# Jakoebly/marl-sc

Measured on AMD Instinct MI355X. Metric: env-steps/sec (agents×envs×steps) at 1/2/4/8 MI355X; CPU ref same host, higher is better.
Workload: dtype int32 state, u64 PCG64, f64 rewards, f32 obs; 1 GPU; InventoryEnvironment.step x 32768 envs/GPU, 8 agents x 64 regions x 5 SKUs (BASELINE configs[2]; configs[3] when N>1); n_envs_per_gpu=32768, agents=8, regions=64, skus=5, episode_length=100, obs_dim_local=34, obs_normalization=meanstd_custom, parallelism=env-shard x1

## Files before the change

### marl-sc_amd/csrc/alloc_kernels.hip

```cpp
#include <hip/hip_runtime.h>
#include <math.h>

#include "env.hpp"
#include "kcommon.hpp"

namespace msc {

#ifndef MSC_AL_CH
#define MSC_AL_CH 8
#endif
constexpr int AL_CH = MSC_AL_CH;
template <int K>
hipError_t launch_alloc_lane_k(const EnvConst& c, const DevEnv* d, const StepIO& io, hipStream_t st);
#ifndef MSC_AL_PRIO
#define MSC_AL_PRIO 3
#endif
#ifndef MSC_AL_PRIO2
#define MSC_AL_PRIO2 1
#endif
#ifndef MSC_AL_PRIO_TAIL
#define MSC_AL_PRIO_TAIL 0
#endif
#ifndef MSC_AL_TAIL_WIN
#define MSC_AL_TAIL_WIN 0
#endif

struct AlLds {
  int rec, inv, shh, qs, out, pen, tab, hm, cl, total;
  __host__ __device__ static AlLds make(int MWL, int MW, int K, int R, bool tab, bool SH) {
    AlLds L{};
    int o = 0;
    L.rec = o; o += AL_CH * ((1 + K + 7) / 8) * 64 * 4;
    L.inv = o; o += MWL * K * 64;
    L.shh = o; o += SH ? MWL * K * 64 : 0;
    L.qs = o;  o += MWL * 64;
    o = (o + 3) & ~3;
    L.out = o; o += MWL * 64 * 2;
    L.pen = o; o += MWL * 64 * 2;
    L.tab = o; o += tab ? (R | 1) * MW * 4 : 0;
    L.hm = o;  o += R;
    L.cl = o;  o += R;
    L.total = o;
    return L;
  }
};
constexpr size_t AL_TAB_MAX = 32 * 1024;

template <int K, int MW, bool DBG, bool TAB, bool SH, bool EXACT, int LPE>
__global__ __launch_bounds__(64) void alloc_lane_kernel(const DevEnv* __restrict__ dp, StepIO io) {
  static_assert(LPE == 1 || LPE == 2 || LPE == 4, "lanes per env");
  static_assert(MW % LPE == 0, "warehouses per lane");
  constexpr int MWL = MW / LPE, EPB = 64 / LPE, LSH = LPE == 1 ? 0 : LPE == 2 ? 1 : 2;
  constexpr int SENT = 0x7fff;
  const EnvConst& c = dp->c;
  const EnvState& s = dp->s;
  const int W = EXACT ? MW : c.W, R = c.R, WK = W * K;
  const int64_t E = c.E;
  const int lane = threadIdx.x, jl = lane & (LPE - 1);
  const int64_t e = (int64_t)blockIdx.x * EPB + (lane >> LSH);
  const bool ev = e < E;
  const msc_step_info info = io.info;
  constexpr bool dbg = DBG;
  constexpr int NVR = Rec<K>::NV;
  if (MSC_AL_PRIO > 0) __builtin_amdgcn_s_setprio(MSC_AL_PRIO);
  auto gw = [&](int i) { return i * LPE + jl; };

  extern __shared__ __attribute__((aligned(16))) int32_t al_lds[];
  const AlLds L = AlLds::make(MWL, MW, K, R, TAB, SH);
  int32_t* Linv = al_lds + L.inv + lane;
  int32_t* Lshh = al_lds + L.shh + lane;
  uint4* Lrec = reinterpret_cast<uint4*>(al_lds + L.rec) + lane;
  double* Lout = reinterpret_cast<double*>(al_lds + L.out) + lane;
  double* Lpen = reinterpret_cast<double*>(al_lds + L.pen) + lane;
  int32_t* Lqs = al_lds + L.qs + lane;
  MSC_GLOBAL int32_t* const incp = gp(s.inc);
  const double2* Ltab = TAB ? reinterpret_cast<const double2*>(al_lds + L.tab) : nullptr;
  const int RS = R | 1;
  const uint32_t* Lhm = reinterpret_cast<const uint32_t*>(al_lds + L.hm);
  const int32_t* Lcl = al_lds + L.cl;
  {
    double2* tw_ = reinterpret_cast<double2*>(al_lds + L.tab);
    if constexpr (TAB) {
      for (int i = lane; i < R * MW; i += 64) {
        const int w = i / R, r = i % R;
        tw_[w * RS + r] = w < W ? make_double2(c.ofT[r * W + w], c.ovT[r * W + w]) : make_double2(0.0, 0.0);
      }
    }
    uint32_t* hm_ = reinterpret_cast<uint32_t*>(al_lds + L.hm);
    int32_t* cl_ = al_lds + L.cl;
    for (int i = lane; i < R; i += 64) {
      hm_[i] = c.home_mask[i];
      cl_[i] = c.closest[i];
    }
  }
  auto tab_at = [&](int r, int w) -> double2 {
    if constexpr (TAB) return Ltab[w * RS + r];
    else return make_double2(gp(c.ofT)[r * W + w], gp(c.ovT)[r * W + w]);
  };

  uint32_t stock[K];
#pragma unroll
  for (int sk = 0; sk < K; sk++) stock[sk] = 0u;
  int invv[MWL][K];
  {
    const int64_t ec = ev ? e : 0;
#pragma unroll
    for (int i = 0; i < MWL; i++) {
      const int w = gw(i), wc = w < W ? w : W - 1;
#pragma unroll
      for (int sk = 0; sk < K; sk++) invv[i][sk] = gp(s.inv)[(int64_t)(wc * K + sk) * E + ec];
    }
  }
#pragma unroll
  for (int i = 0; i < MWL; i++) {
    const int w = gw(i);
#pragma unroll
    for (int sk = 0; sk < K; sk++) {
      const int v = (ev && w < W) ? invv[i][sk] : 0;
      Linv[(i * K + sk) * 64] = v;
      if (SH) Lshh[(i * K + sk) * 64] = 0;
      stock[sk] |= v > 0 ? (1u << i) : 0u;
    }
    Lout[i * 64] = 0.0;
    Lpen[i * 64] = 0.0;
    Lqs[i * 64] = 0;
  }
  __syncthreads();

  const OrderSrc osrc = order_src<NVR>(c, s, io, ev ? e : 0);
  const int n_orders = ev ? osrc.n : 0;
  const int64_t base = ev ? osrc.base : 0, nstep = osrc.nstep, vstep = osrc.vstep;
  const MSC_GLOBAL uint4* src = gp(osrc.src);
  if (dbg && ev && jl == 0 && info.n_orders) info.n_orders[e] = n_orders;
  int wmax = n_orders;
#pragma unroll
  for (int o = 32; o >= 1; o >>= 1) {
    const int v = __shfl_xor(wmax, o);
    wmax = v > wmax ? v : wmax;
  }
  wmax = __builtin_amdgcn_readfirstlane(wmax);

  const int maxwh = c.max_wh, lost_type = c.lost_type, pps = c.pen_per_sku;
  const double alpha = sgpr_d(c.alpha);
  double skw[K], penk[K];
#pragma unroll
  for (int sk = 0; sk < K; sk++) {
    skw[sk] = sgpr_d(c.skw[sk]);
    penk[sk] = sgpr_d(pps ? c.pen[sk] : c.pen_scalar);
  }

  const uint32_t ownw = LPE == 1 ? ~0u : (LPE == 2 ? 0x55555555u : 0x11111111u) << jl;
  int cur = -1, lost_cnt = 0;
  uint32_t hm = 0;
  int hw = -1;
  uint32_t smask = 0;
  int rtot = 0;
  int u[K], dsum[K], shc[K];
#pragma unroll
  for (int sk = 0; sk < K; sk++) u[sk] = dsum[sk] = shc[sk] = 0;
  MSC_GLOBAL int32_t* const shhp = gp(s.sc_shh);
  if (!SH && ev)
    for (int i = 0; i < MWL; i++) {
      const int w = gw(i);
      if (w < W)
        for (int sk = 0; sk < K; sk++) shhp[(int64_t)(w * K + sk) * E + e] = 0;
    }

  auto add_pen = [&](int i, double wt, double upen) {
    Lpen[i * 64] += wt * upen;
    if (dbg && info.lost_sales)
#pragma unroll
      for (int sk = 0; sk < K; sk++) info.lost_sales[e * WK + gw(i) * K + sk] += wt * (double)u[sk];
  };
  auto finalize = [&](int r) {
    if (lost_cnt > 0) {
      double upen = 0.0;
#pragma unroll
      for (int sk = 0; sk < K; sk++) upen += pps ? (double)u[sk] * penk[sk] : ((double)u[sk] * skw[sk]) * penk[sk];
      if (lost_type == MSC_LOST_COST) {
        if constexpr (LPE == 1) {
          double lw = 0.0;
#pragma unroll
          for (int sk = 0; sk < K; sk++) lw += (double)u[sk] * skw[sk];
          double lg[16], mx = -INFINITY;
#pragma unroll
          for (int w = 0; w < 16; w++) {
            lg[w] = -INFINITY;
            if (w < MW && w < W) {
              const double2 t = tab_at(r, w);
              lg[w] = -(t.x * (double)lost_cnt + t.y * lw) / alpha;
              mx = lg[w] > mx ? lg[w] : mx;
            }
          }
          double ex[16];
#pragma unroll
          for (int w = 0; w < 16; w++) ex[w] = (w < MW && w < W) ? exp(lg[w] - mx) : 0.0;
          const double sum = np_sum_f64_16(ex, W);
#pragma unroll
          for (int w = 0; w < MW; w++) {
            const double wt = w < W ? ex[w] / sum : 0.0;
            if (wt != 0.0) add_pen(w, wt, upen);
          }
        }
      } else if (lost_type == MSC_LOST_SHIPMENT && rtot > 0) {
        const double dt = (double)rtot;
        for (uint32_t m = smask; m != 0u; m &= m - 1u) {
          const int i = __builtin_ctz(m);
          add_pen(i, (double)Lqs[i * 64] / dt, upen);
        }
      } else {
        const int cw = Lcl[r];
        if ((cw & (LPE - 1)) == jl) add_pen(cw >> LSH, 1.0, upen);
      }
    }
    for (uint32_t m = smask; m != 0u; m &= m - 1u) Lqs[__builtin_ctz(m) * 64] = 0;
    if (!SH && hw >= 0 && (hw & (LPE - 1)) == jl)
#pragma unroll
      for (int sk = 0; sk < K; sk++) shhp[(int64_t)(hw * K + sk) * E + e] = shc[sk];
    for (uint32_t m = hm & ownw; m != 0u; m &= m - 1u) {
      const int w = __builtin_ctz(m);
#pragma unroll
      for (int sk = 0; sk < K; sk++) incp[(int64_t)(w * K + sk) * E + e] = dsum[sk];
    }
    if (dbg && jl == 0) {
#pragma unroll
      for (int sk = 0; sk < K; sk++) {
        if (info.demand_per_region) info.demand_per_region[(e * R + r) * K + sk] = dsum[sk];
        if (info.unfulfilled_demands) info.unfulfilled_demands[(e * R + r) * K + sk] = u[sk];
      }
      if (info.lost_order_counts) info.lost_order_counts[e * R + r] = lost_cnt;
    }
  };

  uint4 nxt[AL_CH][NVR];
  auto fetch = [&](int win) {
#pragma unroll
    for (int j = 0; j < AL_CH; j++) {
      const int oi = win * AL_CH + j;
#pragma unroll
      for (int v = 0; v < NVR; v++)
        nxt[j][v] = oi < n_orders ? gload4(src, base + oi * nstep + v * vstep) : make_uint4(0u, 0u, 0u, 0u);
    }
  };
  auto publish = [&]() {
#pragma unroll
    for (int j = 0; j < AL_CH; j++)
#pragma unroll
      for (int v = 0; v < NVR; v++) Lrec[(j * NVR + v) * 64] = nxt[j][v];
  };
  fetch(0);
  publish();
  fetch(1);

  const int aps = __builtin_amdgcn_readfirstlane(c.chain_prio ? 16 : c.al_psplit);
  const int psplit = MSC_AL_PRIO > 0 && aps < 16 ? (wmax * aps) >> 4 : -1;
  const bool tail_on = LPE == 1 && __builtin_amdgcn_readfirstlane(c.al_tail) != 0;
  int tail_at = -1;
  int oi = 0;
  for (; oi <= wmax; oi++) {
    if constexpr (LPE == 1) {
      if (tail_on && oi < wmax && (MSC_AL_TAIL_WIN == 0 || oi % AL_CH == 0)) {
        uint32_t any = 0u;
#pragma unroll
        for (int sk = 0; sk < K; sk++) any |= stock[sk];
        if (__builtin_amdgcn_ballot_w64(any != 0u && oi < n_orders) == 0ull) {
          tail_at = oi;
          break;
        }
      }
    }
    if (oi == psplit) __builtin_amdgcn_s_setprio(MSC_AL_PRIO2);
    const int jw = oi % AL_CH;
    if (jw == 0 && oi > 0) {
      publish();
      fetch(oi / AL_CH + 1);
    }
    union {
      uint4 v[NVR];
      uint16_t h[8 * NVR];
    } ur;
#pragma unroll
    for (int v = 0; v < NVR; v++) ur.v[v] = Lrec[(jw * NVR + v) * 64];
    const int r = oi < n_orders ? (int)ur.h[0] : -1;
    if (r != cur) {
#ifndef MSC_AL_ABL_NOFIN
      if (cur >= 0) finalize(cur);
#endif
      cur = r;
      lost_cnt = 0;
#pragma unroll
      for (int sk = 0; sk < K; sk++) u[sk] = dsum[sk] = 0;
      hm = r >= 0 ? Lhm[r] : 0u;
      hw = hm != 0u ? __builtin_ctz(hm) : -1;
      smask = 0u;
      rtot = 0;
#pragma unroll
      for (int sk = 0; sk < K; sk++) shc[sk] = 0;
    }
    if (oi < n_orders) {
    int d[K], rem[K];
    double tw = 0.0;
#pragma unroll
    for (int sk = 0; sk < K; sk++) {
      d[sk] = ur.h[1 + sk];
      rem[sk] = d[sk];
      dsum[sk] += d[sk];
      tw += (double)d[sk] * skw[sk];
    }
    double2 trow[MWL];
#pragma unroll
    for (int i = 0; i < MWL; i++) trow[i] = tab_at(r, TAB ? gw(i) : (gw(i) < W ? gw(i) : W - 1));
    double cost[MWL];
#pragma unroll
    for (int i = 0; i < MWL; i++) cost[i] = gw(i) < W ? trow[i].x + trow[i].y * tw : INFINITY;
    int used = 0;
    bool open = true;
    while (open) {
      uint32_t cand = 0u;
#pragma unroll
      for (int sk = 0; sk < K; sk++) cand |= rem[sk] > 0 ? stock[sk] : 0u;
      if (LPE == 1 && cand == 0u) {
        open = false;
      } else {
      double best = INFINITY;
      int b = LPE == 1 ? 0 : SENT;
#pragma unroll
      for (int i = 0; i < MWL; i++) {
        const bool take = ((cand >> i) & 1u) && cost[i] < best;
        best = take ? cost[i] : best;
        b = take ? gw(i) : b;
      }
      if constexpr (LPE > 1) {
        auto mn = [&](double ob, int o) {
          const bool t = ob < best || (ob == best && o < b);
          best = t ? ob : best;
          b = t ? o : b;
        };
        mn(dpp_x<0>(best), dpp_x<0>(b));
        if constexpr (LPE == 4) mn(dpp_x<1>(best), dpp_x<1>(b));
      }
      if (LPE > 1 && b == SENT) {
        open = false;
      } else {
      const bool own = (b & (LPE - 1)) == jl;
      const int ib = b >> LSH;
      int iv[K], sh[K];
#pragma unroll
      for (int sk = 0; sk < K; sk++) {
        iv[sk] = Linv[(ib * K + sk) * 64];
        sh[sk] = SH ? Lshh[(ib * K + sk) * 64] : 0;
      }
      const bool home_b = (hm >> b) & 1u;
      const double out_b = Lout[ib * 64];
      const int qs_b = Lqs[ib * 64];
      const double2 tb = tab_at(r, b);
      int f[K], fs = 0;
#pragma unroll
      for (int sk = 0; sk < K; sk++) f[sk] = own ? (rem[sk] < iv[sk] ? rem[sk] : iv[sk]) : 0;
      if constexpr (LPE > 1) {
        constexpr int NP = (K + 1) / 2;
        uint32_t pk[NP];
#pragma unroll
        for (int p = 0; p < NP; p++)
          pk[p] = (uint32_t)f[2 * p] | (2 * p + 1 < K ? (uint32_t)f[2 * p + 1] << 16 : 0u);
#pragma unroll
        for (int p = 0; p < NP; p++) {
          pk[p] |= (uint32_t)dpp_x<0>((int)pk[p]);
          if constexpr (LPE == 4) pk[p] |= (uint32_t)dpp_x<1>((int)pk[p]);
        }
#pragma unroll
        for (int sk = 0; sk < K; sk++) f[sk] = (int)((pk[sk / 2] >> (16 * (sk & 1))) & 0xffffu);
      }
      double fw = 0.0;
      bool done = true;
#pragma unroll
      for (int sk = 0; sk < K; sk++) {
        rem[sk] -= f[sk];
        done &= rem[sk] <= 0;
        fs += f[sk];
        fw += (double)f[sk] * skw[sk];
        if (!SH) shc[sk] += home_b ? f[sk] : 0;
      }
      const double oc = fw == tw ? best : tb.x + tb.y * fw;
      if (own) {
#pragma unroll
        for (int sk = 0; sk < K; sk++) {
          const int left = iv[sk] - f[sk];
          stock[sk] &= left > 0 ? ~0u : ~(1u << ib);
          Linv[(ib * K + sk) * 64] = left;
          if (SH) Lshh[(ib * K + sk) * 64] = sh[sk] + (home_b ? f[sk] : 0);
        }
        Lout[ib * 64] = out_b + oc;
        Lqs[ib * 64] = qs_b + fs;
        smask |= 1u << ib;
        if (dbg) {
#pragma unroll
          for (int sk = 0; sk < K; sk++) {
            if (info.shipment_quantities_by_sku) info.shipment_quantities_by_sku[((e * W + b) * R + r) * K + sk] += f[sk];
            if (info.fulfilled_per_warehouse) info.fulfilled_per_warehouse[e * WK + b * K + sk] += f[sk];
          }
          if (info.shipment_counts) info.shipment_counts[(e * W + b) * R + r] += 1;
          if (info.shipment_quantities) info.shipment_quantities[(e * W + b) * R + r] += fs;
        }
      }
      rtot += fs;
      used++;
      open = !(done || used >= maxwh);
#ifdef MSC_AL_ABL_ONEROUND
      open = false;
#endif
      }
      }
    }
    int remor = 0;
#pragma unroll
    for (int sk = 0; sk < K; sk++) {
      remor |= rem[sk];
      u[sk] += rem[sk];
    }
    lost_cnt += remor != 0 ? 1 : 0;
    }
  }

  if constexpr (LPE == 1) {
    if (tail_at >= 0) {
      if (MSC_AL_PRIO_TAIL != 0 && oi < psplit) __builtin_amdgcn_s_setprio(MSC_AL_PRIO2);
      for (; oi <= wmax; oi++) {
        if (MSC_AL_PRIO_TAIL == 0 && oi == psplit) __builtin_amdgcn_s_setprio(MSC_AL_PRIO2);
        const int jw = oi % AL_CH;
        if (jw == 0 && oi > 0) {
          publish();
          fetch(oi / AL_CH + 1);
        }
        union {
          uint4 v[NVR];
          uint16_t h[8 * NVR];
        } ur;
#pragma unroll
        for (int v = 0; v < NVR; v++) ur.v[v] = Lrec[(jw * NVR + v) * 64];
        const int r = oi < n_orders ? (int)ur.h[0] : -1;
        if (r != cur) {
          if (cur >= 0) finalize(cur);
          cur = r;
          lost_cnt = 0;
#pragma unroll
          for (int sk = 0; sk < K; sk++) u[sk] = dsum[sk] = 0;
          hm = r >= 0 ? Lhm[r] : 0u;
          hw = -1;
          smask = 0u;
          rtot = 0;
        }
        if (oi < n_orders) {
          int dor = 0;
#pragma unroll
          for (int sk = 0; sk < K; sk++) {
            const int dq = ur.h[1 + sk];
            dsum[sk] += dq;
            u[sk] += dq;
            dor |= dq;
          }
          lost_cnt += dor != 0 ? 1 : 0;
        }
      }
    }
    if (lane == 0) s.al_tail[blockIdx.x] = tail_at;
  }

  if (!ev) return;
#pragma unroll
  for (int i = 0; i < MWL; i++) {
    const int w = gw(i);
    if (w < W) {
#pragma unroll
      for (int sk = 0; sk < K; sk++) {
        const int64_t g = (int64_t)(w * K + sk) * E + e;
        const int left = Linv[(i * K + sk) * 64];
        s.sc_sht[g] = s.inv[g] - left;
        s.inv[g] = left;
        if (SH) s.sc_shh[g] = Lshh[(i * K + sk) * 64];
      }
      s.sc_pen[w * E + e] = Lpen[i * 64];
      s.sc_out[w * E + e] = Lout[i * 64];
    }
  }
}

static bool shared_homes(const EnvConst& c) { return c.shared_home != 0; }
static size_t alloc_lane_lds_bytes(const EnvConst& c, int MW, int LPE, bool tab) {
  return (size_t)AlLds::make(MW / LPE, MW, c.K, c.R, tab, shared_homes(c)).total * sizeof(int32_t);
}
static bool alloc_tab_in_lds(const EnvConst& c, int MW, int LPE) {
  if ((size_t)(c.R | 1) * MW * 16 <= AL_TAB_MAX) return true;
  const int64_t blocks = (c.E * LPE + 63) / 64;
  return c.demand_type == MSC_DEMAND_EMPIRICAL && blocks <= 256 &&
         alloc_lane_lds_bytes(c, MW, LPE, true) <= 160 * 1024;
}
template <typename F>
static hipError_t alloc_launch(F f, const EnvConst& c, const DevEnv* d, const StepIO& io, hipStream_t st, int lpe,
                               size_t lds) {
  if (lds > 64 * 1024) {
    const hipError_t e = hipFuncSetAttribute((const void*)f, hipFuncAttributeMaxDynamicSharedMemorySize, (int)lds);
    if (e != hipSuccess) return e;
  }
  hipLaunchKernelGGL(f, dim3((unsigned)((c.E * lpe + 63) / 64)), dim3(64), lds, st, d, io);
  return hipGetLastError();
}

static int alloc_lpe(const EnvConst& c, bool dbg, int MW) {
  int lpe = c.alloc_lpe;
  if (lpe != 2 && lpe != 4) lpe = 1;
  if (dbg || shared_homes(c) || c.lost_type == MSC_LOST_COST || MW < 8) lpe = 1;
  return lpe;
}

template <int K, int MW, bool EXACT>
hipError_t launch_alloc_mw(const EnvConst& c, const DevEnv* d, const StepIO& io, hipStream_t st) {
  using KFn = void (*)(const DevEnv*, StepIO);
  const bool dbg = io.has_info != 0;
  const int lpe = alloc_lpe(c, dbg, MW);
  const bool tab = alloc_tab_in_lds(c, MW, lpe);
  const size_t lds = alloc_lane_lds_bytes(c, MW, lpe, tab);
  KFn f;
#define MSC_AL(DB, TB, SHV, LP) (KFn)alloc_lane_kernel<K, MW, DB, TB, SHV, EXACT, LP>
  if constexpr (MW >= 8) {
    if (lpe > 1) {
      f = lpe == 4 ? (tab ? MSC_AL(false, true, false, 4) : MSC_AL(false, false, false, 4))
                   : (tab ? MSC_AL(false, true, false, 2) : MSC_AL(false, false, false, 2));
      return alloc_launch(f, c, d, io, st, lpe, lds);
    }
  }
  if (shared_homes(c))
    f = dbg ? (tab ? MSC_AL(true, true, true, 1) : MSC_AL(true, false, true, 1))
            : (tab ? MSC_AL(false, true, true, 1) : MSC_AL(false, false, true, 1));
  else
    f = dbg ? (tab ? MSC_AL(true, true, false, 1) : MSC_AL(true, false, false, 1))
            : (tab ? MSC_AL(false, true, false, 1) : MSC_AL(false, false, false, 1));
#undef MSC_AL
  return alloc_launch(f, c, d, io, st, 1, lds);
}

template <int K>
hipError_t launch_alloc_lane_k(const EnvConst& c, const DevEnv* d, const StepIO& io, hipStream_t st) {
  if (c.W == 2) return launch_alloc_mw<K, 2, true>(c, d, io, st);
  if (c.W <= 4) return launch_alloc_mw<K, 4, false>(c, d, io, st);
  if (c.W == 8) return launch_alloc_mw<K, 8, true>(c, d, io, st);
  if (c.W < 8) return launch_alloc_mw<K, 8, false>(c, d, io, st);
  if (c.W == 16) return launch_alloc_mw<K, 16, true>(c, d, io, st);
  return launch_alloc_mw<K, 16, false>(c, d, io, st);
}

#ifndef MSC_AL_PART
#define MSC_AL_PART 0
#endif
#define MSC_AL_MW(KV, MWV, EX, KW) KW template hipError_t launch_alloc_mw<KV, MWV, EX>(const EnvConst&, const DevEnv*, const StepIO&, hipStream_t);
#define MSC_AL_EXACT(KV, KW) MSC_AL_MW(KV, 2, true, KW) MSC_AL_MW(KV, 8, true, KW) MSC_AL_MW(KV, 16, true, KW)
#define MSC_AL_MASKED(KV, KW) MSC_AL_MW(KV, 4, false, KW) MSC_AL_MW(KV, 8, false, KW) MSC_AL_MW(KV, 16, false, KW)
#define MSC_AL_K(KV) template hipError_t launch_alloc_lane_k<KV>(const EnvConst&, const DevEnv*, const StepIO&, hipStream_t);
#if MSC_AL_PART == 0
#define MSC_AL_ALL(KV) MSC_AL_EXACT(KV, ) MSC_AL_MASKED(KV, ) MSC_AL_K(KV)
MSC_AL_ALL(1) MSC_AL_ALL(2) MSC_AL_ALL(3) MSC_AL_ALL(4) MSC_AL_ALL(5) MSC_AL_ALL(6) MSC_AL_ALL(7) MSC_AL_ALL(8)
#undef MSC_AL_ALL
#elif MSC_AL_PART == 1
MSC_AL_MASKED(1, extern)
MSC_AL_EXACT(1, )
MSC_AL_K(1)
extern MSC_AL_K(2) extern MSC_AL_K(3) extern MSC_AL_K(4) extern MSC_AL_K(5) extern MSC_AL_K(6) extern MSC_AL_K(7) extern MSC_AL_K(8)
#elif MSC_AL_PART % 2 == 1
MSC_AL_MASKED((MSC_AL_PART + 1) / 2, extern)
MSC_AL_EXACT((MSC_AL_PART + 1) / 2, )
MSC_AL_K((MSC_AL_PART + 1) / 2)
#else
MSC_AL_MASKED(MSC_AL_PART / 2, )
#endif
#undef MSC_AL_K
#undef MSC_AL_MASKED
#undef MSC_AL_EXACT
#undef MSC_AL_MW

#if MSC_AL_PART == 0 || MSC_AL_PART == 1
hipError_t launch_alloc_lane(const EnvConst& c, const DevEnv* d, const StepIO& io, hipStream_t st) {
  switch (c.K) {
    case 1: return launch_alloc_lane_k<1>(c, d, io, st);
    case 2: return launch_alloc_lane_k<2>(c, d, io, st);
    case 3: return launch_alloc_lane_k<3>(c, d, io, st);
    case 4: return launch_alloc_lane_k<4>(c, d, io, st);
    case 5: return launch_alloc_lane_k<5>(c, d, io, st);
    case 6: return launch_alloc_lane_k<6>(c, d, io, st);
    case 7: return launch_alloc_lane_k<7>(c, d, io, st);
    case 8: return launch_alloc_lane_k<8>(c, d, io, st);
    default: return hipErrorInvalidValue;
  }
}
#endif

}
```

### marl-sc_amd/csrc/env_plan.hpp

```cpp
#pragma once
#include "env.hpp"

namespace msc {

inline int order_record_vec4(int K) { return (1 + K + 7) / 8; }
inline bool alloc_scan_supported(int W, int K) { return W <= 16 && K <= 6; }
constexpr int SC_FC_RING = 4;
inline bool alloc_scan_fuse_supported(int W, int K, int RING) { return W <= 8 && K <= 6 && RING <= SC_FC_RING; }
inline int step_b_group_width(int W, int sb_gw) {
  const int gw = W <= 2 ? 2 : W <= 4 ? 4 : W <= 8 ? 8 : W <= 16 ? 16 : 32;
  return sb_gw > gw ? sb_gw : gw;
}

}

#if !defined(__HIP_DEVICE_COMPILE__)
#include <math.h>
#include <stdarg.h>
#include <stdio.h>
#include <stdlib.h>
#include <string.h>

#include <algorithm>
#include <optional>
#include <string>
#include <utility>
#include <vector>

namespace msc {

struct EnvKnobs {
  using Int = std::optional<int>;
  enum class Alloc { unset, lane, group, scan, other };
  enum class EvScope { nofence, device, system };
  enum class EaPrio { normal, low, high };
  std::optional<std::string> demand_impl;
  Alloc alloc_impl = Alloc::unset;
  Int demand_uni, obs_stage, obs_ring_reg, alloc_lpe, alloc_sort, fuse_c, fuse_a, step_c_form, al_prio_split, sc_tab,
      sb_gw, sb_tab, scan_defer, ea, ea_slots, ea_batch, ea_chunk, chain_prio;
  std::optional<double> ea_mem_frac;
  bool pipeline = true;
  bool ev_elide = true;
  EvScope ev_scope = EvScope::nofence;
  EaPrio ea_prio = EaPrio::normal;
};

inline EnvKnobs read_env_knobs(const char* (*lookup)(const char*)) {
  EnvKnobs k;
  auto num = [&](const char* name) { const char* v = lookup(name); return v ? EnvKnobs::Int(atoi(v)) : EnvKnobs::Int(); };
  auto is = [](const char* v, const char* want) { return v && strcmp(v, want) == 0; };
  if (const char* v = lookup("MSC_DEMAND_IMPL")) k.demand_impl = v;
  if (const char* v = lookup("MSC_ALLOC_IMPL"))
    k.alloc_impl = is(v, "group") ? EnvKnobs::Alloc::group : is(v, "lane") ? EnvKnobs::Alloc::lane
                 : is(v, "scan") ? EnvKnobs::Alloc::scan : EnvKnobs::Alloc::other;
  k.demand_uni = num("MSC_DEMAND_UNI");
  k.obs_stage = num("MSC_OBS_STAGE");
  k.obs_ring_reg = num("MSC_OBS_RING_REG");
  k.alloc_lpe = num("MSC_ALLOC_LPE");
  k.alloc_sort = num("MSC_ALLOC_SORT");
  k.fuse_c = num("MSC_FUSE_C");
  k.fuse_a = num("MSC_FUSE_A");
  k.step_c_form = num("MSC_STEP_C_FORM");
  k.al_prio_split = num("MSC_AL_PRIO_SPLIT");
  k.sc_tab = num("MSC_SC_TAB");
  k.sb_gw = num("MSC_SB_GW");
  k.sb_tab = num("MSC_SB_TAB");
  k.scan_defer = num("MSC_SCAN_DEFER");
  k.ea = num("MSC_EA");
  k.ea_slots = num("MSC_EA_SLOTS");
  k.ea_batch = num("MSC_EA_BATCH");
  k.ea_chunk = num("MSC_EA_CHUNK");
  k.chain_prio = num("MSC_CHAIN_PRIO");
  if (const char* v = lookup("MSC_EA_MEM_FRAC")) k.ea_mem_frac = atof(v);
  k.pipeline = !is(lookup("MSC_PIPELINE"), "0");
  k.ev_elide = !is(lookup("MSC_EV_ELIDE"), "0");
  const char* es = lookup("MSC_EV_SCOPE");
  k.ev_scope = is(es, "device") ? EnvKnobs::EvScope::device : is(es, "system") ? EnvKnobs::EvScope::system : EnvKnobs::EvScope::nofence;
  const char* ep = lookup("MSC_EA_PRIO");
  k.ea_prio = is(ep, "low") ? EnvKnobs::EaPrio::low : is(ep, "high") ? EnvKnobs::EaPrio::high : EnvKnobs::EaPrio::normal;
  return k;
}

struct EnvPlan {
  EnvConst c{};
  int nv = 1;
  std::vector<double> hold, pen, ofT, ovT, enlam_o, p_sku, p_skip, enlam_q;
  std::vector<PtrsConst> ptrs_o, ptrs_q;
  std::vector<uint32_t> home_mask;
  std::vector<int32_t> closest, home_of, zeros_wk;
  std::vector<float> zeros_f, ones_f;
  std::vector<int64_t> toff;
  std::vector<uint4> trec;
  bool pipeline = true;
  bool ev_elide = true;
  EnvKnobs::EvScope ev_scope = EnvKnobs::EvScope::nofence;
  EnvKnobs::EaPrio ea_prio = EnvKnobs::EaPrio::normal;
  double ea_frac = 0.25;
  char err[512] = "";
  __attribute__((format(printf, 2, 3))) int fail(const char* fmt, ...) {
    va_list ap;
    va_start(ap, fmt);
    vsnprintf(err, sizeof err, fmt, ap);
    va_end(ap);
    return -1;
  }
};

inline int feature_dim(const msc_env_desc* d, int Lmax) {
  const uint32_t f = d->feature_flags;
  const int K = d->n_skus;
  int n = 0;
  if (f & MSC_F_INVENTORY) n += K + ((f & MSC_F_INVENTORY_AGG) ? 1 : 0);
  if (f & MSC_F_PIPELINE) n += Lmax * K + ((f & MSC_F_PIPELINE_AGG) ? 1 : 0);
  if (f & MSC_F_INCOMING_HOME) n += K + ((f & MSC_F_INCOMING_HOME_AGG) ? 1 : 0);
  if (f & MSC_F_SHIPPED_HOME) n += K;
  if (f & MSC_F_SHIPPED_AWAY) n += K + ((f & MSC_F_SHIPPED_AWAY_AGG) ? 1 : 0);
  if (f & MSC_F_STOCKOUT) n += K;
  if (f & MSC_F_ROLLING_MEAN) n += K + ((f & MSC_F_ROLLING_MEAN_AGG) ? 1 : 0);
  if (f & MSC_F_FORECAST) n += K + ((f & MSC_F_FORECAST_AGG) ? 1 : 0);
  if (f & MSC_F_DAYS_OF_SUPPLY) n += K;
  if (f & MSC_F_NET_POSITION) n += K;
  if (f & MSC_F_DEMAND_VARIABILITY) n += K;
  if (f & MSC_F_DEMAND_HISTORY) n += MSC_HISTORY * K;
  return n;
}

inline int plan_env(const msc_env_desc* d, int64_t n_envs, int n_cus, const EnvKnobs& k, EnvPlan& p) {
  if (!d) return p.fail("null argument");
  if (d->abi_version != MSC_ABI_VERSION) return p.fail("abi_version %d != %d", d->abi_version, MSC_ABI_VERSION);
  const int W = d->n_warehouses, K = d->n_skus, R = d->n_regions;
  if (W < 1 || W > MSC_MAX_W) return p.fail("n_warehouses must be in [1, %d]", MSC_MAX_W);
  if (K < 1 || K > MSC_MAX_K) return p.fail("n_skus must be in [1, %d]", MSC_MAX_K);
  if (R < 1 || R > MSC_MAX_R) return p.fail("n_regions must be in [1, %d]", MSC_MAX_R);
  if (d->episode_length < 1) return p.fail("episode_length must be positive");
  if (n_envs < 1) return p.fail("n_envs must be positive");
  if (d->max_splits < 0 || d->max_splits >= W) return p.fail("max_splits must be < n_warehouses=%d", W);
  const int WK = W * K;
  const bool poisson = d->demand_type == MSC_DEMAND_POISSON, empirical = d->demand_type == MSC_DEMAND_EMPIRICAL;

  int Lmax = 0, lact_max = 0;
  for (int i = 0; i < WK; i++) {
    const int elt = d->expected_lead_times[i];
    if (elt < 1) return p.fail("expected_lead_times must be positive");
    int dev = 0;
    if (d->lead_type == MSC_LEAD_STOCHASTIC) dev = d->max_dev_per_sku ? d->max_deviation[i % K] : d->max_deviation[0];
    if (dev < 0) return p.fail("max_deviation must be non-negative");
    Lmax = elt > Lmax ? elt : Lmax;
    lact_max = elt + dev > lact_max ? elt + dev : lact_max;
  }
  const int RING = lact_max + 1;
  if (RING > MAX_RING) return p.fail("max actual lead time %d exceeds %d", lact_max, MAX_RING - 1);

  EnvConst& c = p.c;
  c = EnvConst{};
  c.W = W; c.K = K; c.R = R; c.T = d->episode_length; c.Lmax = Lmax; c.RING = RING;
  c.F = feature_dim(d, Lmax);
  c.L = c.F + (d->include_warehouse_id ? W : 0);
  c.action_type = d->action_type; c.lead_type = d->lead_type; c.dev_per_sku = d->max_dev_per_sku;
  c.lost_type = d->lost_type; c.scope = d->reward_scope; c.norm = d->obs_norm; c.wid = d->include_warehouse_id;
  c.num_eval = d->num_eval_episodes; c.max_wh = d->max_splits + 1; c.demand_type = d->demand_type;
  c.init_type = d->init_type; c.init_min = d->init_min; c.init_max = d->init_max;
  c.hold_per_sku = d->holding_per_sku; c.pen_per_sku = d->penalty_per_sku;
  c.flags = d->feature_flags; c.E = n_envs; c.scale = d->reward_scale; c.alpha = d->lost_alpha;
  c.hold_scalar = d->holding_per_sku ? 0.0 : d->holding_cost[0];
  c.pen_scalar = d->penalty_per_sku ? 0.0 : d->penalty_cost[0];
  if (c.lost_type == MSC_LOST_COST && !(c.alpha > 0)) return p.fail("cost lost-sales alpha must be > 0");
  if (c.norm == MSC_OBS_MEANSTD && (!d->obs_mean || !d->obs_std)) return p.fail("meanstd needs obs_mean/obs_std");
  if (d->init_type == MSC_INIT_UNIFORM && (d->init_min < 0 || d->init_min > d->init_max))
    return p.fail("uniform initial inventory needs 0 <= min <= max");

  p.hold.assign(K, 0.0), p.pen.assign(K, 0.0);
  for (int s = 0; s < K; s++) {
    p.hold[s] = d->holding_per_sku ? d->holding_cost[s] : 0.0;
    p.pen[s] = d->penalty_per_sku ? d->penalty_cost[s] : 0.0;
  }
  p.ofT.assign((size_t)R * W, 0.0), p.ovT.assign((size_t)R * W, 0.0);
  for (int w = 0; w < W; w++)
    for (int r = 0; r < R; r++) {
      p.ofT[(size_t)r * W + w] = d->outbound_fixed[(size_t)w * R + r];
      p.ovT[(size_t)r * W + w] = d->outbound_variable[(size_t)w * R + r];
    }
  p.home_mask.assign(R, 0u), p.closest.assign(R, 0), p.home_of.assign(W, 0);
  for (int w = 0; w < W; w++) {
    int b = 0;
    for (int r = 1; r < R; r++)
      if (d->distances[(size_t)w * R + r] < d->distances[(size_t)w * R + b]) b = r;
    p.home_mask[b] |= 1u << w;
    p.home_of[w] = b;
  }
  c.shared_home = 0;
  for (int r = 0; r < R; r++) c.shared_home |= __builtin_popcount(p.home_mask[r]) > 1 ? 1 : 0;
  for (int r = 0; r < R; r++) {
    int b = 0;
    for (int w = 1; w < W; w++)
      if (d->distances[(size_t)w * R + r] < d->distances[(size_t)b * R + r]) b = w;
    p.closest[r] = b;
  }
  p.zeros_wk.assign(WK, 0), p.zeros_f.assign(c.F > 0 ? c.F : 1, 0.0f), p.ones_f.assign(c.F > 0 ? c.F : 1, 1.0f);
  p.enlam_o.assign(R, 1.0), p.p_sku.assign(R, 0.0), p.p_skip.assign(R, 0.0), p.enlam_q.assign((size_t)R * K, 1.0);
  p.ptrs_o.assign(R, PtrsConst{}), p.ptrs_q.assign((size_t)R * K, PtrsConst{});
  p.toff.clear(), p.trec.clear();
  const int nv = p.nv = order_record_vec4(K);
  int order_cap = 1;
  int64_t max_count = 1;
  if (poisson) {
    double lam_sum = 0.0;
    for (int r = 0; r < R; r++) {
      const double lo = d->lambda_orders[r];
      if (!(lo > 0.0 && lo < 1e6)) return p.fail("lambda_orders[%d]=%g: must be in (0, 1e6)", r, lo);
      p.enlam_o[r] = exp(-lo);
      p.ptrs_o[r] = ptrs_const_host(lo);
      if (lo >= 10.0) c.demand_ptrs = 1;
      if (lo > 0.0 && lo < 10.0 && p.enlam_o[r] >= 1.0) return p.fail("lambda_orders[%d] too small", r);
      p.p_sku[r] = d->probability_skus[r];
      p.p_skip[r] = ldexp(ceil(ldexp(p.p_sku[r], 53)), -53) - 0x1p-53;
      lam_sum += lo;
      for (int s = 0; s < K; s++) {
        const double lq = d->lambda_quantity[(size_t)r * K + s];
        if (!(lq > 0.0 && lq < 20000.0)) return p.fail("lambda_quantity[%d,%d]=%g: must be in (0, 20000)", r, s, lq);
        p.enlam_q[(size_t)r * K + s] = exp(-lq);
        p.ptrs_q[(size_t)r * K + s] = ptrs_const_host(lq);
        if (lq >= 10.0) c.demand_ptrs = 1;
      }
    }
    const double cap_d = ceil(lam_sum + 12.0 * sqrt(lam_sum + 1.0) + 64.0);
    if (!(cap_d <= (double)MSC_ORDER_CAP_MAX))
      return p.fail("sum of lambda_orders %g: per-step order capacity %.0f exceeds %d records per env", lam_sum, cap_d,
                    MSC_ORDER_CAP_MAX);
    max_count = order_cap = (int)cap_d;
  } else if (empirical) {
    const int rows = d->trace_n_rows;
    if (rows < d->episode_length) return p.fail("trace has %d timesteps < episode_length %d", rows, d->episode_length);
    const int64_t n_ord = d->trace_offsets[rows];
    p.toff.assign(d->trace_offsets, d->trace_offsets + rows + 1);
    p.trec.assign((size_t)(n_ord > 0 ? n_ord : 1) * nv, make_uint4(0, 0, 0, 0));
    for (int64_t j = 0; j < n_ord; j++) {
      uint16_t* h = reinterpret_cast<uint16_t*>(&p.trec[(size_t)j * nv]);
      const int reg = d->trace_regions[j];
      if (reg < 0 || reg >= R) return p.fail("trace region %d out of range", reg);
      h[0] = (uint16_t)reg;
      for (int s = 0; s < K; s++) {
        const int q = d->trace_quantities[j * K + s];
        if (q < 0 || q > 65535) return p.fail("trace quantity %d out of range", q);
        h[1 + s] = (uint16_t)q;
      }
    }
    c.tr_rows = rows;
    max_count = 0;
    for (int i = 0; i < rows; i++) max_count = std::max<int64_t>(max_count, p.toff[i + 1] - p.toff[i]);
  } else {
    return p.fail("unknown demand_type %d", d->demand_type);
  }
  c.order_cap = order_cap;

  if (poisson) {
    c.demand_uni = 1;
    for (int r = 0; r < R; r++) {
      c.demand_uni &= p.enlam_o[r] == p.enlam_o[0] && p.p_skip[r] == p.p_skip[0] ? 1 : 0;
      for (int s = 0; s < K; s++) c.demand_uni &= p.enlam_q[(size_t)r * K + s] == p.enlam_q[0] ? 1 : 0;
    }
    if (k.demand_uni) c.demand_uni &= *k.demand_uni != 0 ? 1 : 0;
    c.uni_thr_o = p.enlam_o[0];
    c.uni_thr_m = p.p_skip[0];
    c.uni_thr_q = p.enlam_q[0];
  }
  if (k.demand_impl && *k.demand_impl != "v3" && *k.demand_impl != "unit")
    return p.fail("MSC_DEMAND_IMPL=%s: accepted values are v3 (the default) and unit", k.demand_impl->c_str());
  c.demand_impl = k.demand_impl && *k.demand_impl == "unit" ? 0 : 9;

  using Alloc = EnvKnobs::Alloc;
  const bool lane = W <= 16 && K <= 8 &&
                    (k.alloc_impl == Alloc::lane || (k.alloc_impl != Alloc::group && poisson && n_envs >= 16384));
  const bool scan = k.alloc_impl == Alloc::scan ? alloc_scan_supported(W, K)
                                                : !lane && k.alloc_impl == Alloc::unset && W <= 8 && alloc_scan_supported(W, K);
  c.alloc_impl = scan ? 2 : lane && k.alloc_impl != Alloc::scan ? 0 : 1;
  c.alloc_lpe = k.alloc_lpe.value_or(0);
  c.alloc_sort = !lane && (k.alloc_sort ? *k.alloc_sort != 0 : empirical) ? 1 : 0;
  c.sort_shift = 0;
  while ((max_count >> c.sort_shift) >= SORT_BUCKETS) c.sort_shift++;
  c.al_psplit = k.al_prio_split && *k.al_prio_split >= 1 && *k.al_prio_split <= 16 ? *k.al_prio_split : 14;
  c.al_tail = 1;

  c.fuse_c = c.alloc_impl == 2 ? (alloc_scan_fuse_supported(W, K, RING) ? 1 : 0)
           : c.alloc_impl == 1 ? (K <= 8 && RING <= 4 ? 1 : 0)
                               : 0;
  if (k.fuse_c) c.fuse_c = c.fuse_c && *k.fuse_c != 0 ? 1 : 0;
  c.fuse_a = c.alloc_impl == 2 && c.fuse_c && d->lead_type != MSC_LEAD_STOCHASTIC && poisson ? 1 : 0;
  if (k.fuse_a) c.fuse_a = c.fuse_a && *k.fuse_a != 0 ? 1 : 0;
  c.scan_defer = k.scan_defer ? (*k.scan_defer != 0 ? 1 : 0) : 1;

  c.sc_tab = k.sc_tab ? (*k.sc_tab != 0 ? 1 : 0) : 1;
  c.sb_gw = k.sb_gw && (*k.sb_gw == 4 || *k.sb_gw == 8 || *k.sb_gw == 16 || *k.sb_gw == 32) ? *k.sb_gw : 0;
  {
    const int ncu = n_cus < 1 ? 256 : n_cus;
    const int gw = step_b_group_width(W, c.sb_gw);
    const int bw = gw >= 16 ? 8 : 4;
    const int64_t blocks = (n_envs * gw + 64 * bw - 1) / (64 * bw), per_cu = (blocks + ncu - 1) / ncu;
    const size_t tab = (size_t)2 * R * W * sizeof(double) + (size_t)R * sizeof(int32_t);
    const size_t blk = (size_t)bw * 2 * 128 * 16 + tab;
    c.sb_tab = tab <= 16 * 1024 ? 1 : (empirical && blk <= 160 * 1024 && (int64_t)blk * per_cu <= 160 * 1024) ? 1 : 0;
    if (k.sb_tab) c.sb_tab = *k.sb_tab != 0 && blk <= 160 * 1024 ? 1 : 0;
  }

  c.obs_stage = (size_t)BS * ((c.W * c.L) | 1) * sizeof(float) <= 80 * 1024 ? (c.W >= 2 ? 2 : 1) : 0;
  if (k.obs_stage) c.obs_stage = c.obs_stage && *k.obs_stage > 0 ? *k.obs_stage : 0;
  if (c.obs_stage > c.W) c.obs_stage = c.W;
  c.obs_ring_reg = k.obs_ring_reg ? *k.obs_ring_reg != 0 : n_envs < 16384 ? 1 : 0;
  c.sc_form = k.step_c_form && *k.step_c_form == 4 ? 4 : 5;

  c.ea_S = 0;
  if (poisson) {
    bool want = d->episode_ahead < 0 ? n_envs <= 8192 : d->episode_ahead > 0;
    if (k.ea) want = *k.ea != 0;
    int S = 16;
    if (d->episode_ahead > 0 && d->episode_ahead < S) S = d->episode_ahead;
    if (k.ea_slots) S = *k.ea_slots;
    S = S < 2 ? 2 : (S > MSC_EA_MAX_S ? MSC_EA_MAX_S : S);
    if (want) {
      double lam_sum = 0.0, draws = 0.0;
      auto per_draw = [](double lam) { return lam < 10.0 ? lam + 1.0 : 8.0; };
      for (int r = 0; r < R; r++) {
        const double lo = d->lambda_orders[r];
        lam_sum += lo;
        double per_order = K;
        for (int s = 0; s < K; s++) per_order += d->probability_skus[r] * per_draw(d->lambda_quantity[(size_t)r * K + s]);
        draws += per_draw(lo) + lo * per_order;
      }
      const double m = lam_sum * d->episode_length;
      draws *= d->episode_length;
      const double cap_d = ceil(m + 12.0 * sqrt(m + 1.0) + 64.0);
      if (cap_d * nv <= (double)INT32_MAX && draws + 12.0 * sqrt(draws + 1.0) < 4294967295.0) {
        c.ea_S = S;
        c.ea_cap = (int64_t)cap_d;
      }
    }
  }
  p.ea_frac = k.ea_mem_frac ? *k.ea_mem_frac : d->ea_mem_fraction > 0.0 ? d->ea_mem_fraction : 0.25;

  p.pipeline = k.pipeline && poisson;
  p.ev_elide = k.ev_elide;
  p.ev_scope = k.ev_scope;
  p.ea_prio = k.ea_prio;
  return 0;
}

struct EaFit {
  int slots;
  int64_t budget;
};
inline EaFit ea_fit_slots(const EnvConst& c, int nv, double ea_frac, int64_t free_bytes) {
  const size_t T = c.T, E = c.E;
  const size_t slot_bytes = sizeof(uint4) * (size_t)nv * c.ea_cap * E + sizeof(int32_t) * (T + 1) * E +
                            sizeof(uint32_t) * T * E + sizeof(int32_t) * E;
  const double budget = ea_frac * (double)(size_t)free_bytes;
  const int64_t fit = (int64_t)(budget / (double)(slot_bytes + 1024 ));
  return {fit < c.ea_S ? (fit < 2 ? 0 : (int)fit) : c.ea_S, (int64_t)budget};
}

struct EaRun {
  int batch = 1, chunk = 50;
  int32_t obs_stage = 0, chain_prio = 0;
};
inline EaRun ea_run_settings(const EnvConst& c, const EnvKnobs& k) {
  EaRun r;
  r.obs_stage = c.obs_stage;
  r.chain_prio = c.chain_prio;
  if (c.ea_S <= 0) return r;
  const int S = c.ea_S;
  int B = c.E <= 8192 ? S / 2 : S / 4;
  B = B > 1 ? B : 1;
  if (k.ea_batch) B = *k.ea_batch;
  r.batch = B < 1 ? 1 : (B > S - 1 ? S - 1 : B);
  if (!(k.obs_stage && *k.obs_stage != 0)) r.obs_stage = 0;
  r.chain_prio = (k.chain_prio && *k.chain_prio == 0) ? 0 : 1;
  int ch = c.E > 8192 ? c.T : 50;
  if (k.ea_chunk) ch = *k.ea_chunk;
  r.chunk = ch < 1 ? 1 : ch;
  return r;
}

struct Packer {
  size_t align;
  size_t end = 0;
  std::vector<char> host;
  std::vector<std::pair<void*, size_t>> fix;
  explicit Packer(size_t a) : align(a) {}
  template <class P>
  void add(P*& field, size_t bytes, const void* src = nullptr) {
    const size_t off = (end + align - 1) & ~(align - 1);
    end = off + bytes;
    if (src) {
      host.resize(end);
      memcpy(host.data() + off, src, bytes);
    }
    fix.emplace_back((void*)&field, off);
  }
  size_t padded() const { return (end + align - 1) & ~(align - 1); }
  void resolve(void* base) const {
    for (const auto& f : fix) {
      char* ptr = static_cast<char*>(base) + f.second;
      memcpy(f.first, &ptr, sizeof ptr);
    }
  }
};

inline void table_layout(const msc_env_desc* d, EnvPlan& p, Packer& t) {
  EnvConst& c = p.c;
  const int K = c.K, R = c.R, W = c.W, WK = W * K;
  const bool stoch = d->lead_type == MSC_LEAD_STOCHASTIC, meanstd = c.norm == MSC_OBS_MEANSTD;
  t.add(c.act_param, sizeof(double) * K, d->action_param);
  t.add(c.init_vals, sizeof(int32_t) * WK, d->init_values ? d->init_values : p.zeros_wk.data());
  t.add(c.hold, sizeof(double) * K, p.hold.data());
  t.add(c.pen, sizeof(double) * K, p.pen.data());
  t.add(c.skw, sizeof(double) * K, d->sku_weights);
  t.add(c.ofT, sizeof(double) * p.ofT.size(), p.ofT.data());
  t.add(c.ovT, sizeof(double) * p.ovT.size(), p.ovT.data());
  t.add(c.inF, sizeof(double) * WK, d->inbound_fixed);
  t.add(c.inV, sizeof(double) * WK, d->inbound_variable);
  t.add(c.enlam_o, sizeof(double) * R, p.enlam_o.data());
  t.add(c.p_sku, sizeof(double) * R, p.p_sku.data());
  t.add(c.p_skip, sizeof(double) * R, p.p_skip.data());
  t.add(c.enlam_q, sizeof(double) * p.enlam_q.size(), p.enlam_q.data());
  t.add(c.ptrs_o, sizeof(PtrsConst) * p.ptrs_o.size(), p.ptrs_o.data());
  t.add(c.ptrs_q, sizeof(PtrsConst) * p.ptrs_q.size(), p.ptrs_q.data());
  t.add(c.elt, sizeof(int32_t) * WK, d->expected_lead_times);
  t.add(c.maxdev, sizeof(int32_t) * (stoch && d->max_dev_per_sku ? K : 1), stoch ? d->max_deviation : p.zeros_wk.data());
  t.add(c.home_mask, sizeof(uint32_t) * R, p.home_mask.data());
  t.add(c.closest, sizeof(int32_t) * R, p.closest.data());
  t.add(c.home_of, sizeof(int32_t) * W, p.home_of.data());
  t.add(c.obs_mean, sizeof(float) * p.zeros_f.size(), meanstd ? d->obs_mean : p.zeros_f.data());
  t.add(c.obs_std, sizeof(float) * p.ones_f.size(), meanstd ? d->obs_std : p.ones_f.data());
  if (c.demand_type == MSC_DEMAND_EMPIRICAL) {
    t.add(c.tr_off, sizeof(int64_t) * p.toff.size(), p.toff.data());
    t.add(c.tr_rec, sizeof(uint4) * p.trec.size(), p.trec.data());
  }
}

inline void arena_layout(const EnvConst& c, EnvState& s, Packer& a) {
  const size_t E = c.E, W = c.W, WK = (size_t)c.W * c.K, RING = c.RING;
  a.add(s.inv, sizeof(int32_t) * WK * E);
  a.add(s.ring_q, sizeof(int32_t) * WK * RING * E);
  a.add(s.ring_l, c.lead_type == MSC_LEAD_STOCHASTIC ? WK * RING * E : 1);
  a.add(s.hist, sizeof(int32_t) * MSC_HISTORY * WK * E);
  a.add(s.inc, sizeof(int32_t) * WK * E);
  a.add(s.fc, sizeof(float) * WK * E);
  a.add(s.rng, sizeof(uint64_t) * 8 * E);
  a.add(s.rbuf, sizeof(uint32_t) * 4 * E);
  a.add(s.rng_pre, sizeof(uint64_t) * 4 * E);
  a.add(s.rbuf_pre, sizeof(uint32_t) * 2 * E);
  a.add(s.t, sizeof(int32_t) * E);
  a.add(s.counter, sizeof(int32_t) * E);
  a.add(s.orig_root, sizeof(uint32_t) * E);
  a.add(s.root, sizeof(uint32_t) * E);
  a.add(s.emp_start, sizeof(int32_t) * E);
  a.add(s.perm, sizeof(int32_t) * E);
  a.add(s.err, sizeof(uint32_t) * 4);
  a.add(s.sc_sht, sizeof(int32_t) * WK * E);
  a.add(s.sc_shh, sizeof(int32_t) * WK * E);
  a.add(s.sc_pen, sizeof(double) * W * E);
  a.add(s.sc_out, sizeof(double) * W * E);
  a.add(s.sc_inb, sizeof(double) * W * E);
}

inline void ea_layout(const EnvConst& c, int nv, EnvState& s, Packer& a) {
  const size_t S = c.ea_S, T = c.T, E = c.E;
  a.add(s.ea_rec, sizeof(uint4) * (size_t)nv * c.ea_cap * S * E);
  a.add(s.ea_off, sizeof(int32_t) * S * (T + 1) * E);
  a.add(s.ea_pos, sizeof(uint32_t) * S * T * E);
  a.add(s.ea_cnt, sizeof(int32_t) * S * E);
}

inline size_t order_record_bytes(const EnvConst& c, int nv) {
  return c.demand_type == MSC_DEMAND_POISSON ? sizeof(uint4) * (size_t)nv * c.order_cap * c.E : 0;
}
inline size_t order_buffer_bytes(const EnvConst& c, int nv) {
  return c.demand_type == MSC_DEMAND_POISSON ? (order_record_bytes(c, nv) + sizeof(int32_t) * c.E + 255) & ~size_t(255) : 0;
}

constexpr int PLAN_N = 26;
inline void plan_values(const EnvConst& c, const EaRun& r, bool pipeline, size_t arena_bytes, size_t order_bytes,
                        int32_t v[PLAN_N]) {
  auto units = [](size_t bytes) { return (int32_t)std::min<size_t>(bytes / 256, INT32_MAX); };
  const int32_t vals[PLAN_N] = {
      c.alloc_impl, c.alloc_sort, c.fuse_a, c.fuse_c, c.sb_tab, c.alloc_impl == 1 ? step_b_group_width(c.W, c.sb_gw) : 0,
      c.ea_S, c.demand_impl, c.demand_uni,
      c.obs_stage, c.obs_ring_reg, c.alloc_lpe, c.sort_shift, c.scan_defer, c.sc_tab, c.sc_form, c.al_psplit,
      c.demand_ptrs, c.order_cap, c.RING, (int32_t)c.ea_cap, r.batch, r.chunk, pipeline ? 1 : 0,
      units(arena_bytes), units(order_bytes)};
  for (int i = 0; i < PLAN_N; i++) v[i] = vals[i];
}

}
#endif
```

Before: 389.1 million agent-steps/s.

## Trim alloc kernel tail finalize work and use 32-bit address math

```diff
diff --git a/marl-sc_amd/csrc/alloc_kernels.hip b/marl-sc_amd/csrc/alloc_kernels.hip
--- a/marl-sc_amd/csrc/alloc_kernels.hip
+++ b/marl-sc_amd/csrc/alloc_kernels.hip
@@ -1,5 +1,7 @@
 #include <hip/hip_runtime.h>
 #include <math.h>
+
+#include <type_traits>
 
 #include "env.hpp"
 #include "kcommon.hpp"
@@ -46,6 +48,27 @@
 };
 constexpr size_t AL_TAB_MAX = 32 * 1024;
 
+__device__ __forceinline__ uint64_t mad_u32(uint32_t a, uint32_t b, uint64_t c) {
+  uint64_t r, carry;
+  asm("v_mad_u64_u32 %0, %1, %2, %3, %4" : "=v"(r), "=s"(carry) : "s"(a), "v"(b), "v"(c));
+  return r;
+}
+
+template <int NV>
+__device__ __forceinline__ void order_bounds(const EnvConst& c, const StepIO& io, const OrderSrc& o, int64_t e, int& room,
+                                             int64_t& spare) {
+  if (c.demand_type == MSC_DEMAND_EMPIRICAL) {
+    room = o.n;
+    spare = 0;
+  } else if (io.ea_slot >= 0) {
+    spare = ((int64_t)io.ea_slot * c.E + e) * c.ea_cap * NV;
+    room = (int)(c.ea_cap - (o.base - spare) / NV);
+  } else {
+    room = c.order_cap;
+    spare = e;
+  }
+}
+
 template <int K, int MW, bool DBG, bool TAB, bool SH, bool EXACT, int LPE>
 __global__ __launch_bounds__(64) void alloc_lane_kernel(const DevEnv* __restrict__ dp, StepIO io) {
   static_assert(LPE == 1 || LPE == 2 || LPE == 4, "lanes per env");
@@ -61,6 +84,10 @@
   const bool ev = e < E;
   const msc_step_info info = io.info;
   constexpr bool dbg = DBG;
+  const uint32_t E32 = (uint32_t)E;
+  auto row_at = [&](MSC_GLOBAL int32_t* p, int row) -> MSC_GLOBAL int32_t* {
+    return p + ((uint64_t)(uint32_t)row * E32 + (uint64_t)e);
+  };
   constexpr int NVR = Rec<K>::NV;
   if (MSC_AL_PRIO > 0) __builtin_amdgcn_s_setprio(MSC_AL_PRIO);
   auto gw = [&](int i) { return i * LPE + jl; };
@@ -140,13 +167,14 @@
   }
   wmax = __builtin_amdgcn_readfirstlane(wmax);
 
-  const int maxwh = c.max_wh, lost_type = c.lost_type, pps = c.pen_per_sku;
+  const int maxwh = c.max_wh, lost_kind = c.lost_type, pps = c.pen_per_sku;
   const double alpha = sgpr_d(c.alpha);
   double skw[K], penk[K];
 #pragma unroll
   for (int sk = 0; sk < K; sk++) {
     skw[sk] = sgpr_d(c.skw[sk]);
     penk[sk] = sgpr_d(pps ? c.pen[sk] : c.pen_scalar);
+    if constexpr (MW == 8 && LPE == 1) asm volatile("" : "+v"(penk[sk]));
   }
 
   const uint32_t ownw = LPE == 1 ? ~0u : (LPE == 2 ? 0x55555555u : 0x11111111u) << jl;
@@ -162,26 +190,32 @@
   if (!SH && ev)
     for (int i = 0; i < MWL; i++) {
       const int w = gw(i);
-      if (w < W)
-        for (int sk = 0; sk < K; sk++) shhp[(int64_t)(w * K + sk) * E + e] = 0;
-    }
-
-  auto add_pen = [&](int i, double wt, double upen) {
+      if (w < W) {
+        MSC_GLOBAL int32_t* p = row_at(shhp, w * K);
+        for (int sk = 0; sk < K; sk++, p += E) *p = 0;
+      }
+    }
+
+  auto add_pen = [&](int i, double wt, double upen, const int (&uu)[K]) {
     Lpen[i * 64] += wt * upen;
     if (dbg && info.lost_sales)
 #pragma unroll
-      for (int sk = 0; sk < K; sk++) info.lost_sales[e * WK + gw(i) * K + sk] += wt * (double)u[sk];
+      for (int sk = 0; sk < K; sk++) info.lost_sales[e * WK + gw(i) * K + sk] += wt * (double)uu[sk];
   };
-  auto finalize = [&](int r) {
+  auto finalize = [&](int r, auto tl) {
+    constexpr bool TL = decltype(tl)::value;
+    const int(&uu)[K] = TL ? dsum : u;
+    int lost_type = lost_kind;
+    asm volatile("" : "+s"(lost_type));
     if (lost_cnt > 0) {
       double upen = 0.0;
 #pragma unroll
-      for (int sk = 0; sk < K; sk++) upen += pps ? (double)u[sk] * penk[sk] : ((double)u[sk] * skw[sk]) * penk[sk];
+      for (int sk = 0; sk < K; sk++) upen += pps ? (double)uu[sk] * penk[sk] : ((double)uu[sk] * skw[sk]) * penk[sk];
       if (lost_type == MSC_LOST_COST) {
         if constexpr (LPE == 1) {
           double lw = 0.0;
 #pragma unroll
-          for (int sk = 0; sk < K; sk++) lw += (double)u[sk] * skw[sk];
+          for (int sk = 0; sk < K; sk++) lw += (double)uu[sk] * skw[sk];
           double lg[16], mx = -INFINITY;
 #pragma unroll
           for (int w = 0; w < 16; w++) {
@@ -199,47 +233,67 @@
 #pragma unroll
           for (int w = 0; w < MW; w++) {
             const double wt = w < W ? ex[w] / sum : 0.0;
-            if (wt != 0.0) add_pen(w, wt, upen);
+            if (wt != 0.0) add_pen(w, wt, upen, uu);
           }
         }
-      } else if (lost_type == MSC_LOST_SHIPMENT && rtot > 0) {
+      } else if (!TL && lost_type == MSC_LOST_SHIPMENT && rtot > 0) {
         const double dt = (double)rtot;
         for (uint32_t m = smask; m != 0u; m &= m - 1u) {
           const int i = __builtin_ctz(m);
-          add_pen(i, (double)Lqs[i * 64] / dt, upen);
+          add_pen(i, (double)Lqs[i * 64] / dt, upen, uu);
         }
       } else {
         const int cw = Lcl[r];
-        if ((cw & (LPE - 1)) == jl) add_pen(cw >> LSH, 1.0, upen);
-      }
-    }
-    for (uint32_t m = smask; m != 0u; m &= m - 1u) Lqs[__builtin_ctz(m) * 64] = 0;
-    if (!SH && hw >= 0 && (hw & (LPE - 1)) == jl)
-#pragma unroll
-      for (int sk = 0; sk < K; sk++) shhp[(int64_t)(hw * K + sk) * E + e] = shc[sk];
-    for (uint32_t m = hm & ownw; m != 0u; m &= m - 1u) {
-      const int w = __builtin_ctz(m);
-#pragma unroll
-      for (int sk = 0; sk < K; sk++) incp[(int64_t)(w * K + sk) * E + e] = dsum[sk];
+        if ((cw & (LPE - 1)) == jl) add_pen(cw >> LSH, 1.0, upen, uu);
+      }
+    }
+    if constexpr (!TL)
+      for (uint32_t m = smask; m != 0u; m &= m - 1u) Lqs[__builtin_ctz(m) * 64] = 0;
+    if constexpr (!SH) {
+      const int w = TL ? (hm != 0u ? __builtin_ctz(hm) : -1) : hw;
+      if (w >= 0 && (w & (LPE - 1)) == jl) {
+        const uint64_t g = (uint64_t)(uint32_t)(w * K) * E32 + (uint64_t)e;
+        if constexpr (!TL) {
+          MSC_GLOBAL int32_t* p = shhp + g;
+#pragma unroll
+          for (int sk = 0; sk < K; sk++, p += E) *p = shc[sk];
+        }
+        MSC_GLOBAL int32_t* p = incp + g;
+#pragma unroll
+        for (int sk = 0; sk < K; sk++, p += E) *p = dsum[sk];
+      }
+    } else {
+      for (uint32_t m = hm & ownw; m != 0u; m &= m - 1u) {
+        MSC_GLOBAL int32_t* p = row_at(incp, __builtin_ctz(m) * K);
+#pragma unroll
+        for (int sk = 0; sk < K; sk++, p += E) *p = dsum[sk];
+      }
     }
     if (dbg && jl == 0) {
 #pragma unroll
       for (int sk = 0; sk < K; sk++) {
         if (info.demand_per_region) info.demand_per_region[(e * R + r) * K + sk] = dsum[sk];
-        if (info.unfulfilled_demands) info.unfulfilled_demands[(e * R + r) * K + sk] = u[sk];
+        if (info.unfulfilled_demands) info.unfulfilled_demands[(e * R + r) * K + sk] = uu[sk];
       }
       if (info.lost_order_counts) info.lost_order_counts[e * R + r] = lost_cnt;
     }
   };
 
   uint4 nxt[AL_CH][NVR];
+  int room;
+  int64_t spare;
+  order_bounds<NVR>(c, io, osrc, ev ? e : 0, room, spare);
+  const int nfetch = n_orders < room ? n_orders : room;
+  const int olast = nfetch > 0 ? nfetch - 1 : 0;
+  const int64_t fbase = nfetch > 0 ? base : spare;
+  const uint32_t nstep32 = (uint32_t)nstep;
   auto fetch = [&](int win) {
 #pragma unroll
     for (int j = 0; j < AL_CH; j++) {
-      const int oi = win * AL_CH + j;
-#pragma unroll
-      for (int v = 0; v < NVR; v++)
-        nxt[j][v] = oi < n_orders ? gload4(src, base + oi * nstep + v * vstep) : make_uint4(0u, 0u, 0u, 0u);
+      const int oi = win * AL_CH + j, oc = oi < olast ? oi : olast;
+      const int64_t at = (int64_t)mad_u32(nstep32, (uint32_t)oc, (uint64_t)fbase);
+#pragma unroll
+      for (int v = 0; v < NVR; v++) nxt[j][v] = gload4(src, at + v * vstep);
     }
   };
   auto publish = [&]() {
@@ -284,7 +338,7 @@
     const int r = oi < n_orders ? (int)ur.h[0] : -1;
     if (r != cur) {
 #ifndef MSC_AL_ABL_NOFIN
-      if (cur >= 0) finalize(cur);
+      if (cur >= 0) finalize(cur, std::false_type{});
 #endif
       cur = r;
       lost_cnt = 0;
@@ -425,6 +479,9 @@
   if constexpr (LPE == 1) {
     if (tail_at >= 0) {
       if (MSC_AL_PRIO_TAIL != 0 && oi < psplit) __builtin_amdgcn_s_setprio(MSC_AL_PRIO2);
+      bool first = true;
+#pragma unroll
+      for (int sk = 0; sk < K; sk++) u[sk] -= dsum[sk];
       for (; oi <= wmax; oi++) {
         if (MSC_AL_PRIO_TAIL == 0 && oi == psplit) __builtin_amdgcn_s_setprio(MSC_AL_PRIO2);
         const int jw = oi % AL_CH;
@@ -440,15 +497,21 @@
         for (int v = 0; v < NVR; v++) ur.v[v] = Lrec[(jw * NVR + v) * 64];
         const int r = oi < n_orders ? (int)ur.h[0] : -1;
         if (r != cur) {
-          if (cur >= 0) finalize(cur);
+          if (cur >= 0) {
+            if (first) {
+#pragma unroll
+              for (int sk = 0; sk < K; sk++) u[sk] += dsum[sk];
+              finalize(cur, std::false_type{});
+            } else {
+              finalize(cur, std::true_type{});
+            }
+          }
+          first = false;
           cur = r;
           lost_cnt = 0;
 #pragma unroll
-          for (int sk = 0; sk < K; sk++) u[sk] = dsum[sk] = 0;
+          for (int sk = 0; sk < K; sk++) dsum[sk] = 0;
           hm = r >= 0 ? Lhm[r] : 0u;
-          hw = -1;
-          smask = 0u;
-          rtot = 0;
         }
         if (oi < n_orders) {
           int dor = 0;
@@ -456,7 +519,6 @@
           for (int sk = 0; sk < K; sk++) {
             const int dq = ur.h[1 + sk];
             dsum[sk] += dq;
-            u[sk] += dq;
             dor |= dq;
           }
           lost_cnt += dor != 0 ? 1 : 0;
diff --git a/marl-sc_amd/csrc/env_plan.hpp b/marl-sc_amd/csrc/env_plan.hpp
--- a/marl-sc_amd/csrc/env_plan.hpp
+++ b/marl-sc_amd/csrc/env_plan.hpp
@@ -134,6 +134,7 @@
   if (R < 1 || R > MSC_MAX_R) return p.fail("n_regions must be in [1, %d]", MSC_MAX_R);
   if (d->episode_length < 1) return p.fail("episode_length must be positive");
   if (n_envs < 1) return p.fail("n_envs must be positive");
+  if (n_envs > INT32_MAX) return p.fail("n_envs must be below 2^31");
   if (d->max_splits < 0 || d->max_splits >= W) return p.fail("max_splits must be < n_warehouses=%d", W);
   const int WK = W * K;
   const bool poisson = d->demand_type == MSC_DEMAND_POISSON, empirical = d->demand_type == MSC_DEMAND_EMPIRICAL;
```

Result: no change. 392.2 million agent-steps/s (median of 6 runs) (+0.8%).
